# MatteoSoldini/metamorphic_testing_of_the_MUSICA_Algorithm_for_x_ray_image_processing

Hardware: AMD Instinct MI355X
Metric: megapixels/sec full MUSICA pipeline (higher is better)
Workload: dtype f32

## Files before the change

metamorphic_testing_of_the_musica_algorithm_for_x_ray_image_processing_amd/build.py:

```python
import os
import subprocess
import sys

HERE = os.path.dirname(os.path.abspath(__file__))
CSRC = os.path.join(HERE, "csrc")
LIB = os.path.join(HERE, "libmusica_hip.so")
CLI = os.path.join(HERE, "musica-standalone")
HIP_SOURCES = ["kernels_pyramid.hip", "kernels_expand_sd.hip", "kernels_analysis.hip", "kernels_gradation.hip", "kernels_clahe.hip", "kernels_bench.hip",
               "kernels_similarity.hip", "kernels_joint.hip", "kernels_displace.hip", "kernels_scales.hip", "kernels_ensemble.hip", "kernels_covariance.hip", "kernels_alteration.hip", "kernels_symmetry.hip", "kernels_export.hip", "musica_ctx.hip", "musica_study.hip"]
CPP_SOURCES = ["musica_io.cpp"]
HEADERS = ["musica_device.h", "kernels_common.h", "exact_math.h", "sdev_parts.h", "grad_parts.h", "launchers.h", "musica_ctx.h", os.path.join("..", "..", "include", "musica.h")]
NO_SLP = {"kernels_analysis.hip", "kernels_expand_sd.hip"}
FLAGS = ["--offload-arch=gfx950", "-O3", "-std=c++17", "-fPIC", "-ffp-contract=off", "-fno-fast-math", "-Wall", "-Wno-unused-function", "-Wno-unused-value", "-Wno-unused-result"]


def _hipcc():
    for cand in (os.environ.get("HIPCC"), "/opt/rocm/bin/hipcc", "hipcc"):
        if cand and (os.path.isabs(cand) and os.path.exists(cand) or not os.path.isabs(cand)):
            return cand
    return "hipcc"


def _stale(target, deps):
    if not os.path.exists(target):
        return True
    t = os.path.getmtime(target)
    return any(os.path.getmtime(d) > t for d in deps if os.path.exists(d))


def build(force=False, verbose=False):
    hipcc = _hipcc()
    objdir = os.path.join(HERE, "build")
    os.makedirs(objdir, exist_ok=True)
    headers = [os.path.normpath(os.path.join(CSRC, h)) for h in HEADERS]
# ... 105 lines not shown
```

metamorphic_testing_of_the_musica_algorithm_for_x_ray_image_processing_amd/csrc/exact_math.h:

```cpp
#pragma once

#include <math.h>
#include <stdint.h>

#if defined(__HIPCC__)
#define MUSICA_HD __host__ __device__ __forceinline__
#else
#define MUSICA_HD static inline
#endif

MUSICA_HD float musica_div25(float x) {
    const float y = 0.04f;
    const float q = x * y;
    const float r = fmaf(-25.0f, q, x);
    return r == r ? fmaf(r, y, q) : q;
}

MUSICA_HD int musica_noise_bin_exact(float cur) {
    if (cur != cur) return 0;
    if (cur == 0.0f) return 0;
    const float a = cur / 0.1f;
    if (a > 1.0f) return 0;
    return (int)(a * 2048.0f + 0.5f);
}
// ... 19 lines not shown
    return fmaf(r, h, s);
}
__device__ __forceinline__ bool musica_sqrt_core_ok(float x) {
    const uint32_t u = __float_as_uint(x);
    return u == 0u || (u - 0x0D800000u) < (0x7F800000u - 0x0D800000u);
}
__device__ __forceinline__ void musica_sqrt8(float s[8]) {
    uint32_t mx = 0u, mn = 0xFFFFFFFFu;
#pragma unroll
    for (int j = 0; j < 8; j++) {
        const uint32_t u = __float_as_uint(s[j]);
        mx = max(mx, u);
        mn = min(mn, u - 1u);
    }
    const bool ok = mx < 0x7F800000u && mn >= 0x0D800000u - 1u;
    if (__builtin_expect(ok, 1)) {
#pragma unroll
        for (int j = 0; j < 8; j++) s[j] = musica_sqrt_core(s[j]);
    } else {
#pragma unroll
        for (int j = 0; j < 8; j++) s[j] = sqrtf(s[j]);
    }
}
__device__ __forceinline__ float musica_sqrt(float x) {
    const float s = musica_sqrt_core(x);
    if (__builtin_expect(!musica_sqrt_core_ok(x), 0)) return sqrtf(x);
    return s;
}
#endif
```

metamorphic_testing_of_the_musica_algorithm_for_x_ray_image_processing_amd/csrc/kernels_analysis.hip:

```cpp
#include <stdlib.h>
#include <algorithm>
#include "kernels_common.h"
#include "exact_math.h"
#include "launchers.h"
#include "sdev_parts.h"

namespace musica {

__global__ void k_clear(uint32_t* __restrict__ minmax, uint32_t* __restrict__ noise_hist, uint32_t* __restrict__ grad_hist,
                        uint32_t* __restrict__ clahe_hist, int batch, uint32_t* __restrict__ grad_hist_b, uint32_t* __restrict__ gzero) {
    const int i = blockIdx.x * blockDim.x + threadIdx.x;
    const int nh = batch * 4 * MUSICA_NOISE_BINS, gh = batch * MUSICA_GRAD_BINS;
    const int ch = clahe_hist ? batch * MUSICA_CLAHE_TILES * MUSICA_CLAHE_TILES * MUSICA_CLAHE_BINS : 0;
    if (minmax && i < batch) { minmax[kMinMaxStride * i] = 0xFFFFFFFFu; minmax[kMinMaxStride * i + kMaxWord] = 0u; }
    if (noise_hist && i < nh) noise_hist[i] = 0u;
    if (grad_hist && i < gh) grad_hist[i] = 0u;
    if (grad_hist_b && i < gh) grad_hist_b[i] = 0u;
    if (gzero && i < batch) gzero[i] = 0u;
    if (i < ch) clahe_hist[i] = 0u;
}

__device__ __forceinline__ uint32_t wave_min(uint32_t v) {
#pragma unroll
    for (int o = 32; o >= 1; o >>= 1) v = min(v, (uint32_t)__shfl_xor((int)v, o));
// ... 104 lines not shown
    }
}

__device__ __forceinline__ bool same_float(float a, float b) { return __float_as_uint(a) == __float_as_uint(b) || (a != a && b != b); }
__global__ __launch_bounds__(256) void k_selftest_sqrt(unsigned long long* __restrict__ bad) {
    const uint64_t stride = (uint64_t)gridDim.x * blockDim.x;
    unsigned long long b0 = 0, b1 = 0, b2 = 0;
    for (uint64_t grp = (uint64_t)blockIdx.x * blockDim.x + threadIdx.x; grp < (1ull << 29); grp += stride) {
        float want[8], s[8], z[8];
#pragma unroll
        for (int j = 0; j < 8; j++) {
            const float x = __uint_as_float((uint32_t)(grp * 8 + j));
            want[j] = sqrtf(x);
            s[j] = x;
            z[j] = j == (int)(grp & 7) ? 0.0f : x;
            if (!same_float(musica_sqrt(x), want[j])) b0++;
        }
        musica_sqrt8(s);
        musica_sqrt8(z);
#pragma unroll
        for (int j = 0; j < 8; j++) {
            if (!same_float(s[j], want[j])) b1++;
            if (!same_float(z[j], j == (int)(grp & 7) ? 0.0f : want[j])) b2++;
        }
    }
    if (b0) atomicAdd(&bad[0], b0);
    if (b1) atomicAdd(&bad[1], b1);
    if (b2) atomicAdd(&bad[2], b2);
}
__global__ __launch_bounds__(256) void k_selftest_norm(unsigned long long* __restrict__ bad) {
    if (blockIdx.y < blockIdx.x) return;
    const float minv = (float)blockIdx.x, maxv = (float)blockIdx.y;
    const NormK nk = make_norm(minv, maxv);
    unsigned long long b = 0;
    for (uint32_t v = threadIdx.x; v < 65536u; v += blockDim.x)
        if (!same_float(norm_px(v, nk), norm_px(v, minv, maxv - minv))) b++;
    if (b) atomicAdd(&bad[3], b);
}

__global__ __launch_bounds__(256) void k_normalize(const uint16_t* __restrict__ px, float* __restrict__ out, int N, int pitch,
                                                   size_t plane, const uint32_t* __restrict__ minmax, int min_chain_exact) {
    const int img = blockIdx.z;
    float minv, maxv;
    chain_scalars(minmax, img, min_chain_exact, minv, maxv);
    const NormK nk = make_norm(minv, maxv);
    const uint16_t* p = px + (size_t)img * N * N;
// ... 150 lines not shown
        const unsigned long long other = __shfl_xor(k, o);
        k = other > k ? other : k;
    }
    const int lane = threadIdx.x & 63, wv = threadIdx.x >> 6, nw = (blockDim.x + 63) >> 6;
    if (lane == 0) scratch[wv] = k;
    __syncthreads();
    unsigned long long r = 0ull;
    for (int i = 0; i < nw; i++) r = scratch[i] > r ? scratch[i] : r;
    __syncthreads();
    return r;
}

__device__ __forceinline__ void noise_curves_block(int level, int img, const uint32_t* __restrict__ hist, size_t hist_stride,
                                                   musica_hist_max_point* __restrict__ maxpts, DevCurve* __restrict__ curves,
                                                   const musica_contrast_params* __restrict__ cparams, int levels,
                                                   DevCurveLut* __restrict__ luts, const uint32_t* __restrict__ minmax, int min_chain_exact,
                                                   int* __restrict__ thr090) {
    __shared__ unsigned long long scratch[16];
    if (thr090 && level == levels - 1 && threadIdx.x == 255) {
        float minv, maxv;
        chain_scalars(minmax, img, min_chain_exact, minv, maxv);
        thr090[img] = norm_threshold_090(minv, maxv - minv);
    }
    __shared__ float sx[kCurveCap];
    __shared__ int sbucket[kCurveCap];
    __shared__ int sok;
    musica_hist_max_point mp;
    mp.maxValue = 0; mp.maxBin = 0;
    if (level <= MUSICA_CNR_LEVEL) {
        const uint32_t* h = hist + (size_t)img * hist_stride + (size_t)level * MUSICA_NOISE_BINS;
        unsigned long long k = 0ull;
        for (int i = threadIdx.x; i < MUSICA_NOISE_BINS; i += blockDim.x) {
            const unsigned long long ki = argmax_key(h[i], (uint32_t)i);
            k = ki > k ? ki : k;
        }
        k = block_max_u64(k, scratch);
        if (k) { mp.maxValue = (uint32_t)(k >> 32); mp.maxBin = 0xFFFFFFFFu - (uint32_t)(k & 0xFFFFFFFFull); }
    }
    DevCurve* c = curves + (size_t)img * levels + level;
    __shared__ float cx[kCurveCap], cy[kCurveCap];
    __shared__ int s_mono;
    if (threadIdx.x == 0) maxpts[(size_t)img * levels + level] = mp;
    const float low = cparams[level].lowContrastFactor, high = cparams[level].highContrastFactor;
    const bool constant = (low == 1.0f);
    const int npts = constant ? 2 : 33;
    if ((int)threadIdx.x < kCurveCap) {
        const int i = threadIdx.x;
        float x = 0.0f, y = 0.0f;
        if (constant) {
            if (i == 0) { x = 0.0f; y = high; }
            if (i == 1) { x = 1.0f; y = high; }
        } else if (i < 33) {
            const float p = (float)mp.maxBin * (1.0f / (float)MUSICA_NOISE_BINS) * kMaxNoiseValue;
            const int seg = i / 11;
            const uint32_t k = (uint32_t)(i - seg * 11);
            if (seg == 0) bezier_point(0.0f, 1.0f, p * 4.0f / 5.0f, low, p, low, k, x, y);
            else if (seg == 1) bezier_point(p, low, p * 6.0f / 5.0f, low, p * 7.0f / 5.0f, low * 4.0f / 5.0f, k, x, y);
            else bezier_point(p * 7.0f / 5.0f, low * 4.0f / 5.0f, p * 2.0f, 1.0f, 1.0f, 1.0f, k, x, y);
        }
        cx[i] = x;
        cy[i] = y;
    }
    __syncthreads();
    curve_store_parallel(c, cx, cy, &s_mono, npts, 0.0f, 0.0f, 0.0f);
    if (level >= MUSICA_COARSER_LEVELS_START) return;
    __syncthreads();
    DevCurveLut* lut = luts + (size_t)img * MUSICA_COARSER_LEVELS_START + level;
    const int count = npts;
    const float range = cx[kLutTailFirst - 1] * 1.25f;
    const float inv_w = (float)kLutBuckets / range;
    __shared__ int scoarse[kCurveCap];
    if (threadIdx.x == 0) sok = (s_mono && count == kLutPoints && range > 0.0f && inv_w < 3.0e38f && cx[0] == 0.0f) ? 1 : 0;
    if ((int)threadIdx.x < kCurveCap) {
        const float x = cx[threadIdx.x];
        sx[threadIdx.x] = x;
        const float kf = x * inv_w;
        sbucket[threadIdx.x] = ((int)threadIdx.x < count && kf < (float)kLutBuckets) ? (int)kf : kLutBuckets;
        const float cf = fminf(x * 256.0f, (float)(kLutCoarse - 1));
        scoarse[threadIdx.x] = (int)cf;
    }
    __syncthreads();
    if ((int)threadIdx.x < count) {
        const bool inside = sbucket[threadIdx.x] < kLutBuckets;
        if (inside != ((int)threadIdx.x < kLutTailFirst)) sok = 0;
    }
    for (int k = threadIdx.x; k < kLutBuckets + kLutCoarse; k += blockDim.x) {
        const bool fine = k < kLutBuckets;
        const int kb = fine ? k : k - kLutBuckets;
        const int first = fine ? 0 : kLutTailFirst;
        int jlo = first, inb = 0;
        float xa = __builtin_huge_valf(), xb = __builtin_huge_valf();
        for (int i = first; i < count && i < kCurveCap; i++) {
            const int b = fine ? sbucket[i] : scoarse[i];
            if (b < kb) jlo++;
            else if (b == kb) {
                if (inb == 0) xa = sx[i];
                else if (inb == 1) xb = sx[i];
                inb++;
            }
        }
        if (inb > 2) sok = 0;
        lut->bucket[k] = make_float4(__int_as_float(jlo * 16), xa, xb, 0.0f);
    }
    if ((int)threadIdx.x <= kLutPoints) {
        const int j = threadIdx.x;
        float4 sg = make_float4(0.0f, 0.0f, 0.0f, 0.0f);
        if (j == 0) sg = make_float4(cx[0], cy[0], 0.0f, 0.0f);
        else if (j < count) sg = make_float4(cx[j - 1], cy[j - 1], (cy[j] - cy[j - 1]) / (cx[j] - cx[j - 1]), 0.0f);
        lut->seg[j] = sg;
    }
    __syncthreads();
    if (threadIdx.x == 0) {
        lut->inv_w = inv_w;
        lut->ok = (uint32_t)sok;
        lut->pad0 = lut->pad1 = 0;
    }
}

__global__ __launch_bounds__(256) void k_noise_curves(const uint32_t* __restrict__ hist, size_t hist_stride,
                                                      musica_hist_max_point* __restrict__ maxpts, DevCurve* __restrict__ curves,
                                                      const musica_contrast_params* __restrict__ cparams, int levels,
                                                      DevCurveLut* __restrict__ luts, const uint32_t* __restrict__ minmax, int min_chain_exact,
                                                      int* __restrict__ thr090, int lev0) {
    noise_curves_block(lev0 + (int)blockIdx.x, blockIdx.y, hist, hist_stride, maxpts, curves, cparams, levels, luts, minmax, min_chain_exact, thr090);
}

__global__ __launch_bounds__(256) void k_curves_cnr(const uint32_t* __restrict__ hist, size_t hist_stride,
                                                    musica_hist_max_point* __restrict__ maxpts, DevCurve* __restrict__ curves,
                                                    const musica_contrast_params* __restrict__ cparams, int levels,
                                                    DevCurveLut* __restrict__ luts, const float* __restrict__ sdev, float* __restrict__ cnr,
                                                    int S, int pitch, size_t plane, int tiles_x, const uint32_t* __restrict__ minmax,
                                                    int min_chain_exact, int* __restrict__ thr090, int lev0) {
    const int img = blockIdx.y;
    const int nlev = levels - lev0;
    if ((int)blockIdx.x < nlev) {
        noise_curves_block(lev0 + (int)blockIdx.x, img, hist, hist_stride, maxpts, curves, cparams, levels, luts, minmax, min_chain_exact, thr090);
        return;
    }
// ... 237 lines not shown
```

metamorphic_testing_of_the_musica_algorithm_for_x_ray_image_processing_amd/csrc/kernels_common.h:

```cpp
#pragma once

#include "musica_device.h"
#include "exact_math.h"

namespace musica {

__device__ __forceinline__ float from_left_lane(float v) {
    const int s = __builtin_bit_cast(int, v);
    return __builtin_bit_cast(float, __builtin_amdgcn_update_dpp(s, s, 0x138, 0xF, 0xF, true));
}
__device__ __forceinline__ float from_right_lane(float v) {
    const int s = __builtin_bit_cast(int, v);
    return __builtin_bit_cast(float, __builtin_amdgcn_update_dpp(s, s, 0x130, 0xF, 0xF, true));
}

typedef int v4i __attribute__((ext_vector_type(4)));
typedef float v4f __attribute__((ext_vector_type(4)));
typedef float v2f __attribute__((ext_vector_type(2)));
__device__ v4f llvm_buffer_load_v4f32(v4i rsrc, int voffset, int soffset, int aux) __asm("llvm.amdgcn.raw.buffer.load.v4f32");
__device__ v2f llvm_buffer_load_v2f32(v4i rsrc, int voffset, int soffset, int aux) __asm("llvm.amdgcn.raw.buffer.load.v2f32");
__device__ float llvm_buffer_load_f32(v4i rsrc, int voffset, int soffset, int aux) __asm("llvm.amdgcn.raw.buffer.load.f32");
__device__ void llvm_buffer_store_v4f32(v4f data, v4i rsrc, int voffset, int soffset, int aux) __asm("llvm.amdgcn.raw.buffer.store.v4f32");
__device__ short llvm_buffer_load_i16(v4i rsrc, int voffset, int soffset, int aux) __asm("llvm.amdgcn.raw.buffer.load.i16");
__device__ void llvm_buffer_store_i16(short data, v4i rsrc, int voffset, int soffset, int aux) __asm("llvm.amdgcn.raw.buffer.store.i16");
// ... 196 lines not shown
    return 0.0f;
}

__device__ __forceinline__ void curve_finish(DevCurve* c) {
    const int count = (int)c->count;
    uint32_t mono = 1;
    for (int i = 0; i < kCurveCap; i++) {
        if (i + 1 < count) {
            c->m[i] = (c->y[i + 1] - c->y[i]) / (c->x[i + 1] - c->x[i]);
            if (!(c->x[i] <= c->x[i + 1])) mono = 0;
        } else {
            c->m[i] = 0.0f;
        }
        if (i >= count) {
            c->x[i] = 0.0f;
            c->y[i] = 0.0f;
        }
    }
    if (count > 0 && !(c->x[0] == c->x[0])) mono = 0;
    if (count > 63) mono = 0;
    c->monotone = mono;
}

__device__ __forceinline__ float interpolate(float from, float to, float percent) {
    float difference = to - from;
    return from + (difference * percent);
}

__device__ __forceinline__ void generate_curve(DevCurve* c, uint32_t& n, float sx, float sy, float mx, float my,
                                               float ex, float ey, uint32_t steps) {
    for (uint32_t i = 0; i < steps; i++) {
        float t = (float)i / 10.0f;
        float xa = interpolate(sx, mx, t);
        float ya = interpolate(sy, my, t);
        float xb = interpolate(mx, ex, t);
        float yb = interpolate(my, ey, t);
        c->x[n] = interpolate(xa, xb, t);
        c->y[n] = interpolate(ya, yb, t);
        n++;
    }
}

__device__ __forceinline__ void bezier_point(float sx, float sy, float mx, float my, float ex, float ey, uint32_t k, float& x, float& y) {
    const float t = (float)k / 10.0f;
    const float xa = interpolate(sx, mx, t);
    const float ya = interpolate(sy, my, t);
    const float xb = interpolate(mx, ex, t);
    const float yb = interpolate(my, ey, t);
    x = interpolate(xa, xb, t);
    y = interpolate(ya, yb, t);
}

__device__ __forceinline__ void curve_store_parallel(DevCurve* c, const float* sx, const float* sy, int* s_mono, int count, float t0, float ta, float t1) {
    const int i = threadIdx.x;
    if (i == 0) *s_mono = 1;
    __syncthreads();
    if (i < kCurveCap) {
        float m = 0.0f;
        if (i + 1 < count) {
            m = (sy[i + 1] - sy[i]) / (sx[i + 1] - sx[i]);
            if (!(sx[i] <= sx[i + 1])) *s_mono = 0;
        }
        if (i == 0 && count > 0 && !(sx[0] == sx[0])) *s_mono = 0;
        c->x[i] = sx[i];
        c->y[i] = sy[i];
        c->m[i] = m;
    }
    __syncthreads();
    if (i == 0) {
        c->count = (uint32_t)count;
        c->monotone = (*s_mono && count <= 63) ? 1u : 0u;
        c->t0 = t0; c->ta = ta; c->t1 = t1;
        c->pad = 0;
    }
}
// ... 21 lines not shown
```

metamorphic_testing_of_the_musica_algorithm_for_x_ray_image_processing_amd/csrc/kernels_pyramid.hip:

```cpp
#include <stdlib.h>
#include "kernels_common.h"
#include "sdev_parts.h"
#include "launchers.h"

#ifndef MUSICA_PYRAMID_SD_ONLY
#define MUSICA_PYRAMID_FULL 1
#endif

namespace musica {

struct LaneCfg {
    int c;
    bool active;
    bool left_mirror;
    bool last_active;
    bool lane0, lane63;
    uint32_t off;
    uint32_t off_l;
    uint32_t off_r;
    uint32_t coff;
    uint32_t coff_l;
    uint32_t coff_r;
};

// ... 487 lines not shown
    r = c > highCnr ? highFactor : r;
    r = c < lowCnr ? lowFactor : r;
    return r;
}
__device__ __forceinline__ float nr_factor(float c, float lowCnr, float lowFactor, float highCnr, float highFactor) {
    if (c < lowCnr) return lowFactor;
    else if (c > highCnr) return highFactor;
    const float m = (highFactor - lowFactor) / (highCnr - lowCnr);
    return m * c + lowFactor;
}

template <int GAIN>
__device__ __forceinline__ float gain_of(float s, float high, const CurveLds& t) {
    if (GAIN == GAIN_CONST) return high;
    if (GAIN == GAIN_RANGE) {
        if (s == 0.0f) return high;
        if (s >= 0.0f && s <= 1.0f) return 0.0f * s + high;
        return 0.0f;
    }
    return curve_eval(t, s);
}

struct LutLds {
    float4 bucket[kLutBuckets + kLutCoarse];
    float4 seg[kLutPoints + 1];
    float inv_w;
    uint32_t ok;
};
template <bool LUTOK>
__device__ __forceinline__ float curve_eval_lut(const CurveLds& t, const LutLds& lut, float s) {
    if (!LUTOK) return curve_eval(t, s);
    const float sf = fminf(s, 2.0f);
    const float kf = sf * lut.inv_w;
    const bool in_fine = kf < (float)kLutBuckets;
    const float tsel = in_fine ? kf : fminf(sf * 256.0f, (float)(kLutCoarse - 1));
    const int idx = max((int)tsel + (in_fine ? 0 : kLutBuckets), 0);
    const float4 e = lut.bucket[idx];
    const int joff = __float_as_int(e.x) + (e.y < sf ? 16 : 0) + (e.z < sf ? 16 : 0);
    const float4 g = *reinterpret_cast<const float4*>(reinterpret_cast<const char*>(lut.seg) + joff);
    const float r = g.z * (sf - g.x) + g.y;
    return sf < 0.0f ? 0.0f : r;
}

constexpr int kChSlots = 4, kChCopies = 2;
#ifndef MUSICA_SD_W
#define MUSICA_SD_W 3
#endif
#ifndef MUSICA_SD_CH_W
#define MUSICA_SD_CH_W 2
#endif
struct BRow {
    float v[8];
    float e0, e1;
};
__device__ __forceinline__ void sdev_from_band(const BRow& r0, const BRow& r1, const BRow& r2, const BRow& r3, const BRow& r4, bool lane0, bool lane63, float (&s)[8]) {
    float q[8];
#pragma unroll
    for (int j = 0; j < 8; j++) q[j] = sum5(r0.v[j] * r0.v[j], r1.v[j] * r1.v[j], r2.v[j] * r2.v[j], r3.v[j] * r3.v[j], r4.v[j] * r4.v[j]);
    const float qe0 = sum5(r0.e0 * r0.e0, r1.e0 * r1.e0, r2.e0 * r2.e0, r3.e0 * r3.e0, r4.e0 * r4.e0);
    const float qe1 = sum5(r0.e1 * r0.e1, r1.e1 * r1.e1, r2.e1 * r2.e1, r3.e1 * r3.e1, r4.e1 * r4.e1);
    float a6 = from_left_lane(q[6]), a7 = from_left_lane(q[7]);
    float b0 = from_right_lane(q[0]), b1 = from_right_lane(q[1]);
    if (lane0) { a6 = qe0; a7 = qe1; }
    if (lane63) { b0 = qe0; b1 = qe1; }
    s[0] = sum5(a6, a7, q[0], q[1], q[2]);
    s[1] = sum5(a7, q[0], q[1], q[2], q[3]);
    s[2] = sum5(q[0], q[1], q[2], q[3], q[4]);
    s[3] = sum5(q[1], q[2], q[3], q[4], q[5]);
    s[4] = sum5(q[2], q[3], q[4], q[5], q[6]);
    s[5] = sum5(q[3], q[4], q[5], q[6], q[7]);
    s[6] = sum5(q[4], q[5], q[6], q[7], b0);
    s[7] = sum5(q[5], q[6], q[7], b0, b1);
#pragma unroll
    for (int j = 0; j < 8; j++) s[j] = musica_div25(s[j]);
    musica_sqrt8(s);
}
template <int GAIN, bool NR, bool GH, bool LUTOK, bool CNR48, bool CH = false, bool SD = false>
__device__ __forceinline__ bool expand_march(const ExpandArgs& a, const CurveLds& tab, const LutLds& lut, uint32_t* lh, int img, uint32_t* lc = nullptr,
                                             uint32_t tx0 = 0u, uint32_t ty0 = 0u) {
    constexpr int kGhCopies = 4, kGhStride = MUSICA_GRAD_BINS + 8;
    const float nr_m = (a.highFactor - a.lowFactor) / (a.highCnr - a.lowCnr);
    const int lane = threadIdx.x & 63;
    const Tile tile = xcd_tile(a.swz);
    const int seg = __builtin_amdgcn_readfirstlane((int)(tile.segblock * kWavesPerBlock + (threadIdx.x >> 6)));
    const int k0 = seg * a.rows_per_wave;
    bool saw_zero = false;
    if (k0 < a.Sc) {
    const int k1 = min(k0 + a.rows_per_wave, a.Sc);
    const int S = a.S;
    const int cnrScale = GH ? 8 : a.cnrScale;
    const Buf bb = make_buf(a.band + (size_t)img * a.plane, a.plane * 4);
    const Buf sb = make_buf((GAIN != GAIN_CONST ? a.sdev : a.band) + (size_t)img * a.plane, a.plane * 4);
    const Buf ob = make_buf(a.recon + (size_t)img * a.plane, a.plane * 4);
    const Buf pb = make_buf(a.prev + (size_t)img * a.cplane, a.cplane * 4);
    const Buf wb = !GH ? bb : make_buf(a.le090 + (size_t)img * a.Sc * (S / 8), (size_t)a.Sc * (S / 8) * 2);
    const float* cnr = NR ? a.cnr + (size_t)img * a.cnrPlane : nullptr;
    const LaneCfg g = make_cfg(tile.strip, lane, S);
    const uint32_t rb = (uint32_t)a.pitch * 4u, crb = (uint32_t)a.cpitch * 4u;
    const uint32_t moff = g.off == kOob ? kOob : (uint32_t)g.c >> 2, mrb = (uint32_t)S >> 2;
    const int cxs[2] = {g.active ? g.c / cnrScale : 0, g.active ? (g.c + 4) / cnrScale : 0};
    const uint32_t border = 100u, lim = (uint32_t)S - border;
    uint32_t colin = 0u;
    if (GH) {
#pragma unroll
        for (int j = 0; j < 8; j++)
            if (g.active && (uint32_t)(g.c + j) > border && (uint32_t)(g.c + j) < lim) colin |= 1u << j;
    }
    uint32_t* lhc = lh + (GH ? (lane & (kGhCopies - 1)) * kGhStride : 0);
    const float fS = (float)S;
    uint32_t chx = 0u;
    if (CH) {
#pragma unroll
        for (int j = 0; j < 8; j++) chx |= (min(f2u((float)(g.c + j) / fS * (float)MUSICA_CLAHE_TILES) - tx0, 1u)) << j;
    }
    uint32_t* lcc = CH ? lc + (lane & (kChCopies - 1)) * (kChSlots * MUSICA_CLAHE_BINS) : nullptr;

    auto row_phase = [&](const int ph, float* b, const float* src, const float* sd, const float* low, const float* f, const uint32_t le_t,
                         const int kk, const uint32_t w_cnr, const uint32_t w_dark_or_ramp, const bool one_ramp, const bool one_dark) __attribute__((always_inline)) {
#pragma unroll
        for (int j = 0; j < 8; j++) {
            float p = src[j] * (GAIN == GAIN_CURVE ? curve_eval_lut<LUTOK>(tab, lut, sd[j]) : gain_of<GAIN>(GAIN != GAIN_CONST ? sd[j] : 0.0f, a.high, tab));
            if (NR) p = p * f[j];
            b[j] = low[j] + p;
        }
        store8_nt(ob, g.off + (uint32_t)(2 * kk + ph) * rb, b);
        if (GH) {
            const uint32_t dark = le_t >> (8 * ph);
            const uint32_t y = (uint32_t)(2 * kk + ph);
            const uint32_t m = (y > border && y < lim) ? colin : 0u;
            const uint32_t chy = CH ? min(f2u((float)y / fS * (float)MUSICA_CLAHE_TILES) - ty0, 1u) : 0u;
#pragma unroll
            for (int j = 0; j < 8; j++) {
                const float cur = b[j];
                saw_zero = saw_zero || (cur == 0.0f);
                const uint32_t bin = min((uint32_t)(int)fminf(fmaxf(cur * (float)MUSICA_GRAD_BINS, -1.0f), 2048.0f), (uint32_t)MUSICA_GRAD_BINS);
                const bool le090 = ((dark >> j) & 1u) != 0u;
                const uint32_t w = ((m >> j) & 1u) * (le090 ? w_dark_or_ramp : w_cnr);
                atomicAdd(&lhc[bin], w);
                if (CH) {
                    const float scaled = cur * (float)(MUSICA_CLAHE_BINS - 1) + 0.5f;
                    const bool inrange = scaled > -1.0f && scaled < (float)MUSICA_CLAHE_BINS;
                    if (((m >> j) & 1u) && inrange && (one_ramp || (one_dark && le090)))
                        atomicAdd(&lcc[((((chx >> j) & 1u) * 2u + chy) * MUSICA_CLAHE_BINS) + (uint32_t)(int)scaled], 1u);
                }
            }
        }
    };
    if constexpr (SD) {
        const uint32_t off_e = g.lane0 ? g.off_l : g.off_r;
        auto load_brow = [&](BRow& r, const int y, const bool wanted) __attribute__((always_inline)) {
            const uint32_t row_off = (wanted && y >= 0 && y < S) ? (uint32_t)y * rb : kOob;
            load8(r.v, bb, (g.off + row_off) | ((g.off | row_off) & kOob));
            const float2 e = bload2(bb, (off_e + row_off) | ((off_e | row_off) & kOob));
            r.e0 = e.x; r.e1 = e.y;
        };
        CRow c0, c1, cn;
        load_crow(c0, pb, (uint32_t)coarse_of_fine(2 * k0 - 2, S) * crb, g);
        load_crow(c1, pb, (uint32_t)k0 * crb, g);
// ... 122 lines not shown
                }
            }
        }
        const CnrClass kc = classify_cnr(cnr_pair);
        const uint32_t w_cnr = kc.ramp ? kc.w_ramp : 0u, w_dark_or_ramp = kc.ramp ? kc.w_ramp : (kc.high ? 100u : 0u);
        const float r6 = cnr_pair / 6.0f;
        const bool one_ramp = CH && kc.ramp && (((r6 * r6) * (r6 * r6)) * r6 == 1.0f);
        const bool one_dark = CH && !kc.ramp && kc.high;
        row_phase(0, be, be, se, lowE, fe, le, k, w_cnr, w_dark_or_ramp, one_ramp, one_dark);
        load8(be, bb, goff_n + (uint32_t)(2 * kn) * rb);
        if (GAIN != GAIN_CONST) load8(se, sb, goff_n + (uint32_t)(2 * kn) * rb);
        row_phase(1, bo, bo, so, lowO, fo, le, k, w_cnr, w_dark_or_ramp, one_ramp, one_dark);
        le = le_n;
    }
    }
    return saw_zero;
}

template <int GAIN, bool NR, bool GH, int W = 1, bool CH = false, bool SD = false>
__global__ __launch_bounds__(kBlockThreads, W) void k_expand_fast(ExpandArgs a) {
    __shared__ CurveLds tab;
    __shared__ __attribute__((aligned(16))) LutLds lut;
    constexpr int kGhCopies = 4, kGhStride = MUSICA_GRAD_BINS + 8;
    __shared__ uint32_t lh[GH ? kGhCopies * kGhStride : 1];
    __shared__ uint32_t lc[CH ? kChCopies * kChSlots * MUSICA_CLAHE_BINS : 1];
    const int img = blockIdx.z;
    if (GH)
        for (int i = threadIdx.x; i < kGhCopies * kGhStride; i += blockDim.x) lh[i] = 0u;
    uint32_t tx0 = 0u, ty0 = 0u;
    if (CH) {
        for (int i = threadIdx.x; i < kChCopies * kChSlots * MUSICA_CLAHE_BINS; i += blockDim.x) lc[i] = 0u;
        const Tile t = xcd_tile(a.swz);
        tx0 = f2u((float)(t.strip * kStripCols) / (float)a.S * (float)MUSICA_CLAHE_TILES);
        ty0 = f2u((float)(t.segblock * kWavesPerBlock * a.rows_per_wave * 2) / (float)a.S * (float)MUSICA_CLAHE_TILES);
    }
    if (GAIN == GAIN_CURVE) {
        const DevCurve* cv = a.curves + (size_t)img * a.curve_stride;
        const DevCurveLut* lv = a.luts + (size_t)img * MUSICA_COARSER_LEVELS_START;
        curve_to_lds(tab, cv);
        for (int i = threadIdx.x; i < kLutBuckets + kLutCoarse; i += blockDim.x) lut.bucket[i] = lv->bucket[i];
        for (int i = threadIdx.x; i <= kLutPoints; i += blockDim.x) lut.seg[i] = lv->seg[i];
        if (threadIdx.x == 0) { lut.inv_w = lv->inv_w; lut.ok = lv->ok; }
        __syncthreads();
    }
    const bool lut_ok = GAIN != GAIN_CURVE || __builtin_amdgcn_readfirstlane((int)lut.ok) != 0;
    const bool cnr48 = !NR || GH || a.cnrScale == 4 || a.cnrScale == 8;
    bool saw_zero;
    if (lut_ok && cnr48) saw_zero = expand_march<GAIN, NR, GH, true, true, CH, SD>(a, tab, lut, lh, img, lc, tx0, ty0);
    else if (lut_ok) saw_zero = expand_march<GAIN, NR, GH, true, NR && !GH ? false : true, CH, SD>(a, tab, lut, lh, img, lc, tx0, ty0);
    else if (cnr48) saw_zero = expand_march<GAIN, NR, GH, GAIN != GAIN_CURVE, true, CH, SD>(a, tab, lut, lh, img, lc, tx0, ty0);
    else saw_zero = expand_march<GAIN, NR, GH, GAIN != GAIN_CURVE, NR && !GH ? false : true, CH, SD>(a, tab, lut, lh, img, lc, tx0, ty0);
    if (GH) {
        if (saw_zero) atomicOr(&a.gzero[img], 1u);
        __syncthreads();
        uint32_t* gh = a.ghist + (size_t)img * MUSICA_GRAD_BINS;
        for (int i = threadIdx.x; i < MUSICA_GRAD_BINS; i += blockDim.x) {
            uint32_t v = 0u;
#pragma unroll
            for (int k = 0; k < kGhCopies; k++) v += lh[k * kGhStride + i];
            if (v) atomicAdd(&gh[i], v);
        }
        if (CH) {
            uint32_t* ch = a.chist + (size_t)img * MUSICA_CLAHE_TILES * MUSICA_CLAHE_TILES * MUSICA_CLAHE_BINS;
            for (int i = threadIdx.x; i < kChSlots * MUSICA_CLAHE_BINS; i += blockDim.x) {
                const uint32_t slot = (uint32_t)i / MUSICA_CLAHE_BINS, tx = tx0 + (slot >> 1), ty = ty0 + (slot & 1u);
                uint32_t v = 0u;
#pragma unroll
                for (int k = 0; k < kChCopies; k++) v += lc[k * kChSlots * MUSICA_CLAHE_BINS + i];
                if (v && tx < (uint32_t)MUSICA_CLAHE_TILES && ty < (uint32_t)MUSICA_CLAHE_TILES)
                    atomicAdd(&ch[(tx * MUSICA_CLAHE_TILES + ty) * MUSICA_CLAHE_BINS + ((uint32_t)i % MUSICA_CLAHE_BINS)], v);
            }
        }
    }
}

__device__ __forceinline__ void curve_to_lds_2d(CurveLds& tab, const DevCurve* __restrict__ src) {
    const int tid = threadIdx.y * blockDim.x + threadIdx.x;
    for (int i = tid; i < kCurveCap; i += blockDim.x * blockDim.y) {
        tab.x[i] = src->x[i]; tab.y[i] = src->y[i]; tab.m[i] = src->m[i];
    }
    if (tid == 0) { tab.count = src->count; tab.monotone = src->monotone; }
}
// ... 260 lines not shown
```

metamorphic_testing_of_the_musica_algorithm_for_x_ray_image_processing_amd/csrc/musica_device.h:

```cpp
#pragma once

#include <hip/hip_runtime.h>
#include <stdint.h>

#include "../../include/musica.h"

namespace musica {

__device__ constexpr float W0 = 0.1f, W1 = 0.25f, W2 = 0.3f, W3 = 0.25f, W4 = 0.1f;

constexpr int kLaneCols = 8;
constexpr int kStripCols = 64 * kLaneCols;
constexpr int kWavesPerBlock = 4;
constexpr int kBlockThreads = 64 * kWavesPerBlock;

constexpr float kMaxNoiseValue = 0.1f;
constexpr float kMaxCnrValue = 256.0f;
constexpr int kHistArea = 16;
constexpr int kMinMaxStride = 32;
constexpr int kMaxWord = 16;
constexpr int kCurveCap = 64;

struct DevCurve {
    float x[kCurveCap];
    float y[kCurveCap];
    float m[kCurveCap];
    uint32_t count;
    uint32_t monotone;
    float t0, ta, t1;
    uint32_t pad;
};

constexpr int kLutBuckets = 256;
constexpr int kLutCoarse = 258;
constexpr int kLutTailFirst = 23;
constexpr int kLutPoints = 33;
struct DevCurveLut {
    float inv_w;
    uint32_t ok;
    uint32_t pad0, pad1;
    float4 bucket[kLutBuckets + kLutCoarse];
    float4 seg[kLutPoints + 1];
};

struct LevelDesc {
    int S;
    int pitch;
    size_t plane;
};

constexpr int kSdevRunLevelsMax = 4;
struct SdevRunLevel {
    const float* band;
    float* sdev;
    uint32_t* hist;
    size_t plane;
    int S, pitch, strips, first;
    int rows;
    int blocks;
};
struct SdevRunLevels {
    SdevRunLevel l[kSdevRunLevelsMax];
    int n;
    int swz;
// ... 23 lines not shown
```

metamorphic_testing_of_the_musica_algorithm_for_x_ray_image_processing_amd/csrc/sdev_parts.h:

```cpp
#pragma once

#include "kernels_common.h"
#include "exact_math.h"

namespace musica {

constexpr int kHistCopies = 3;
constexpr int kHistCopyStride = MUSICA_NOISE_BINS + 8;
constexpr int kHistLdsWords = kHistCopies * kHistCopyStride + 64;
__device__ __forceinline__ void hist_lds_clear(uint32_t* lh) {
    for (int i = threadIdx.x; i < kHistLdsWords; i += blockDim.x) lh[i] = 0u;
}
__device__ __forceinline__ void hist_lds_flush(const uint32_t* lh, uint32_t* __restrict__ gh) {
    for (int i = threadIdx.x; i < MUSICA_NOISE_BINS; i += blockDim.x) {
        uint32_t v = 0u;
#pragma unroll
        for (int k = 0; k < kHistCopies; k++) v += lh[k * kHistCopyStride + i];
        if (v) atomicAdd(&gh[i], v);
    }
}

struct SRow {
    float q[8];
    float l0, l1;
// ... 65 lines not shown
    acc = acc + d;
    acc = acc + e;
    return acc;
}

__device__ __forceinline__ void sdev_values(const SRow& r0, const SRow& r1, const SRow& r2, const SRow& r3, const SRow& r4, const SCfg& g, float (&s)[8]) {
    float q[8];
#pragma unroll
    for (int j = 0; j < 8; j++) q[j] = sum5(r0.q[j], r1.q[j], r2.q[j], r3.q[j], r4.q[j]);
    const float ql0 = sum5(r0.l0, r1.l0, r2.l0, r3.l0, r4.l0), ql1 = sum5(r0.l1, r1.l1, r2.l1, r3.l1, r4.l1);
    const float qh0 = sum5(r0.h0, r1.h0, r2.h0, r3.h0, r4.h0), qh1 = sum5(r0.h1, r1.h1, r2.h1, r3.h1, r4.h1);
    float a6 = from_left_lane(q[6]), a7 = from_left_lane(q[7]);
    float b0 = from_right_lane(q[0]), b1 = from_right_lane(q[1]);
    if (g.lane0) { a6 = ql0; a7 = ql1; }
    if (g.lane63) { b0 = qh0; b1 = qh1; }
    s[0] = sum5(a6, a7, q[0], q[1], q[2]);
    s[1] = sum5(a7, q[0], q[1], q[2], q[3]);
    s[2] = sum5(q[0], q[1], q[2], q[3], q[4]);
    s[3] = sum5(q[1], q[2], q[3], q[4], q[5]);
    s[4] = sum5(q[2], q[3], q[4], q[5], q[6]);
    s[5] = sum5(q[3], q[4], q[5], q[6], q[7]);
    s[6] = sum5(q[4], q[5], q[6], q[7], b0);
    s[7] = sum5(q[5], q[6], q[7], b0, b1);
#pragma unroll
    for (int j = 0; j < 8; j++) s[j] = musica_div25(s[j]);
    musica_sqrt8(s);
}
template <bool A8>
__device__ __forceinline__ void sdev_store(const float (&s)[8], const SCfg& g, float* __restrict__ drow, const Buf& db, uint32_t row_off) {
    if (A8) {
        bstore4(db, (g.off0 + row_off) | (g.off0 & kOob), make_float4(s[0], s[1], s[2], s[3]));
        bstore4(db, (g.off1 + row_off) | (g.off1 & kOob), make_float4(s[4], s[5], s[6], s[7]));
    } else if (g.valid == 8) {
        *reinterpret_cast<float4*>(drow + g.c) = make_float4(s[0], s[1], s[2], s[3]);
        *reinterpret_cast<float4*>(drow + g.c + 4) = make_float4(s[4], s[5], s[6], s[7]);
    } else {
#pragma unroll
        for (int j = 0; j < 8; j++)
            if (j < g.valid) drow[g.c + j] = s[j];
    }
}

template <bool HIST, bool A8>
__device__ __forceinline__ void sdev_row(const SRow& r0, const SRow& r1, const SRow& r2, const SRow& r3, const SRow& r4, const SCfg& g, int S,
                                         int y, int cov, float* __restrict__ drow, const Buf& db, uint32_t row_off, uint32_t* lh,
                                         unsigned long long (&alive)[8], const unsigned long long (&start)[8], bool store = true) {
    float s[8];
    sdev_values(r0, r1, r2, r3, r4, g, s);
    if (store) sdev_store<A8>(s, g, drow, db, row_off);
// ... 140 lines not shown
```

Measured before the change: 115,200.

## Key curve LUT on float exponent bits and fuse div25+sqrt range check

Replaces the two-level bucket LUT for the gain curve (fine buckets scaled by inv_w plus a coarse tail) with a single table indexed by the float's bit pattern shifted right, starting at a per-curve base key. This removes a float multiply, a compare and a select from each curve evaluation, and the kernel copies only the used entries into LDS. The LDS table grows to 1160 entries, which may lower occupancy. It also adds musica_rms25_8, which checks the range once for all 8 values before doing the exact divide-by-25 and fast sqrt, and drops the clamp on the histogram bin by shifting the histogram base by one word so a bin of -1 stays in bounds.

```diff
diff --git a/metamorphic_testing_of_the_musica_algorithm_for_x_ray_image_processing_amd/build.py b/metamorphic_testing_of_the_musica_algorithm_for_x_ray_image_processing_amd/build.py
--- a/metamorphic_testing_of_the_musica_algorithm_for_x_ray_image_processing_amd/build.py
+++ b/metamorphic_testing_of_the_musica_algorithm_for_x_ray_image_processing_amd/build.py
@@ -9,7 +9,7 @@
 HIP_SOURCES = ["kernels_pyramid.hip", "kernels_expand_sd.hip", "kernels_analysis.hip", "kernels_gradation.hip", "kernels_clahe.hip", "kernels_bench.hip",
                "kernels_similarity.hip", "kernels_joint.hip", "kernels_displace.hip", "kernels_scales.hip", "kernels_ensemble.hip", "kernels_covariance.hip", "kernels_alteration.hip", "kernels_symmetry.hip", "kernels_export.hip", "musica_ctx.hip", "musica_study.hip"]
 CPP_SOURCES = ["musica_io.cpp"]
-HEADERS = ["musica_device.h", "kernels_common.h", "exact_math.h", "sdev_parts.h", "grad_parts.h", "launchers.h", "musica_ctx.h", os.path.join("..", "..", "include", "musica.h")]
+HEADERS = ["musica_device.h", "kernels_common.h", "exact_math.h", "curve_lut.h", "sdev_parts.h", "grad_parts.h", "launchers.h", "musica_ctx.h", os.path.join("..", "..", "include", "musica.h")]
 NO_SLP = {"kernels_analysis.hip", "kernels_expand_sd.hip"}
 FLAGS = ["--offload-arch=gfx950", "-O3", "-std=c++17", "-fPIC", "-ffp-contract=off", "-fno-fast-math", "-Wall", "-Wno-unused-function", "-Wno-unused-value", "-Wno-unused-result"]
 
diff --git a/metamorphic_testing_of_the_musica_algorithm_for_x_ray_image_processing_amd/csrc/curve_lut.h b/metamorphic_testing_of_the_musica_algorithm_for_x_ray_image_processing_amd/csrc/curve_lut.h
--- /dev/null
+++ b/metamorphic_testing_of_the_musica_algorithm_for_x_ray_image_processing_amd/csrc/curve_lut.h
@@ -0,0 +1,99 @@
+#pragma once
+
+#include <math.h>
+#include <stdint.h>
+#include <string.h>
+
+#include "exact_math.h"
+
+namespace musica {
+
+constexpr int kLutPoints = 33;
+constexpr int kLutShift = 17;
+constexpr int kLutKeyTop = 0x40000000 >> kLutShift;
+constexpr int kLutCap = 1160;
+
+MUSICA_HD int32_t musica_float_bits(float f) {
+#if defined(__HIP_DEVICE_COMPILE__)
+    return __float_as_int(f);
+#else
+    int32_t i;
+    memcpy(&i, &f, sizeof i);
+    return i;
+#endif
+}
+MUSICA_HD float musica_bits_float(int32_t i) {
+#if defined(__HIP_DEVICE_COMPILE__)
+    return __int_as_float(i);
+#else
+    float f;
+    memcpy(&f, &i, sizeof f);
+    return f;
+#endif
+}
+MUSICA_HD float musica_lut_clamp(float s) { return s < 2.0f ? s : 2.0f; }
+MUSICA_HD int musica_lut_key_clamped(float sf) { return musica_float_bits(sf) >> kLutShift; }
+MUSICA_HD int musica_lut_key(float s) { return musica_lut_key_clamped(musica_lut_clamp(s)); }
+MUSICA_HD int musica_lut_index(int key, int base) { return (key > base ? key : base) - base; }
+
+MUSICA_HD float interpolate(float from, float to, float percent) {
+    float difference = to - from;
+    return from + (difference * percent);
+}
+MUSICA_HD void bezier_point(float sx, float sy, float mx, float my, float ex, float ey, uint32_t k, float& x, float& y) {
+    const float t = (float)k / 10.0f;
+    const float xa = interpolate(sx, mx, t);
+    const float ya = interpolate(sy, my, t);
+    const float xb = interpolate(mx, ex, t);
+    const float yb = interpolate(my, ey, t);
+    x = interpolate(xa, xb, t);
+    y = interpolate(ya, yb, t);
+}
+MUSICA_HD void musica_contrast_point(uint32_t maxBin, float low, int i, float& x, float& y) {
+    const float p = (float)maxBin * (1.0f / 2048.0f) * 0.1f;
+    const int seg = i / 11;
+    const uint32_t k = (uint32_t)(i - seg * 11);
+    if (seg == 0) bezier_point(0.0f, 1.0f, p * 4.0f / 5.0f, low, p, low, k, x, y);
+    else if (seg == 1) bezier_point(p, low, p * 6.0f / 5.0f, low, p * 7.0f / 5.0f, low * 4.0f / 5.0f, k, x, y);
+    else bezier_point(p * 7.0f / 5.0f, low * 4.0f / 5.0f, p * 2.0f, 1.0f, 1.0f, 1.0f, k, x, y);
+}
+
+MUSICA_HD int musica_lut_base(const float* x) { return musica_lut_key(x[1]) - 1; }
+MUSICA_HD int musica_lut_entries(int base) {
+    const int n = kLutKeyTop - base + 1;
+    return (base >= 0 && n <= kLutCap) ? n : 0;
+}
+MUSICA_HD int musica_lut_slot(float x, int base) { return musica_lut_index(musica_lut_key(x), base); }
+constexpr int kLutSlotSentinel = 0x7FFFFFFF;
+template <class F4>
+MUSICA_HD int musica_lut_entry(const float* x, const int* b, int count, int k, F4& e) {
+    int jlo = 0;
+    for (int step = 32; step >= 1; step >>= 1) {
+        const int probe = jlo + step;
+        if (probe <= count && b[probe - 1] < k) jlo = probe;
+    }
+    const bool ia = b[jlo] == k, ib = b[jlo + 1] == k, ic = b[jlo + 2] == k;
+    e.x = musica_bits_float(jlo * 16);
+    e.y = ia ? x[jlo] : (float)INFINITY;
+    e.z = ib ? x[jlo + 1] : (float)INFINITY;
+    e.w = 0.0f;
+    return (ia ? 1 : 0) + (ib ? 1 : 0) + (ic ? 1 : 0);
+}
+template <class F4>
+MUSICA_HD void musica_lut_segment(const float* x, const float* y, int count, int j, F4& sg) {
+    sg.x = sg.y = sg.z = sg.w = 0.0f;
+    if (j == 0) { sg.x = x[0]; sg.y = y[0]; }
+    else if (j < count) { sg.x = x[j - 1]; sg.y = y[j - 1]; sg.z = (y[j] - y[j - 1]) / (x[j] - x[j - 1]); }
+}
+template <class F4>
+MUSICA_HD float musica_lut_eval(const F4* bucket, const F4* seg, int base, float s) {
+    const float sf = musica_lut_clamp(s);
+    const int idx = musica_lut_index(musica_lut_key_clamped(sf), base);
+    const F4 e = *reinterpret_cast<const F4*>(reinterpret_cast<const char*>(bucket) + (uint32_t)idx * 16u);
+    const int joff = musica_float_bits(e.x) + (e.y < sf ? 16 : 0) + (e.z < sf ? 16 : 0);
+    const F4 g = *reinterpret_cast<const F4*>(reinterpret_cast<const char*>(seg) + joff);
+    const float r = g.z * (sf - g.x) + g.y;
+    return sf < 0.0f ? 0.0f : r;
+}
+
+}
diff --git a/metamorphic_testing_of_the_musica_algorithm_for_x_ray_image_processing_amd/csrc/exact_math.h b/metamorphic_testing_of_the_musica_algorithm_for_x_ray_image_processing_amd/csrc/exact_math.h
--- a/metamorphic_testing_of_the_musica_algorithm_for_x_ray_image_processing_amd/csrc/exact_math.h
+++ b/metamorphic_testing_of_the_musica_algorithm_for_x_ray_image_processing_amd/csrc/exact_math.h
@@ -65,6 +65,27 @@
         for (int j = 0; j < 8; j++) s[j] = sqrtf(s[j]);
     }
 }
+__device__ __forceinline__ void musica_rms25_8(float s[8]) {
+    uint32_t mx = 0u, mn = 0xFFFFFFFFu;
+#pragma unroll
+    for (int j = 0; j < 8; j++) {
+        const uint32_t u = __float_as_uint(s[j]);
+        mx = max(mx, u);
+        mn = min(mn, u - 1u);
+    }
+    const bool ok = mx < 0x7F800000u && mn >= 0x10000000u - 1u;
+    if (__builtin_expect(ok, 1)) {
+#pragma unroll
+        for (int j = 0; j < 8; j++) {
+            const float q = s[j] * 0.04f;
+            const float r = fmaf(-25.0f, q, s[j]);
+            s[j] = musica_sqrt_core(fmaf(r, 0.04f, q));
+        }
+    } else {
+#pragma unroll
+        for (int j = 0; j < 8; j++) s[j] = sqrtf(s[j] / 25.0f);
+    }
+}
 __device__ __forceinline__ float musica_sqrt(float x) {
     const float s = musica_sqrt_core(x);
     if (__builtin_expect(!musica_sqrt_core_ok(x), 0)) return sqrtf(x);
diff --git a/metamorphic_testing_of_the_musica_algorithm_for_x_ray_image_processing_amd/csrc/kernels_analysis.hip b/metamorphic_testing_of_the_musica_algorithm_for_x_ray_image_processing_amd/csrc/kernels_analysis.hip
--- a/metamorphic_testing_of_the_musica_algorithm_for_x_ray_image_processing_amd/csrc/kernels_analysis.hip
+++ b/metamorphic_testing_of_the_musica_algorithm_for_x_ray_image_processing_amd/csrc/kernels_analysis.hip
@@ -150,6 +150,26 @@
         for (int j = 0; j < 8; j++) {
             if (!same_float(s[j], want[j])) b1++;
             if (!same_float(z[j], j == (int)(grp & 7) ? 0.0f : want[j])) b2++;
+        }
+        const float repl[3] = {0.0f, __uint_as_float(0x03800000u) , __uint_as_float(0x7F800000u)};
+        float want25[8], r[8];
+#pragma unroll
+        for (int j = 0; j < 8; j++) {
+            r[j] = __uint_as_float((uint32_t)(grp * 8 + j));
+            want25[j] = sqrtf(r[j] / 25.0f);
+        }
+        musica_rms25_8(r);
+#pragma unroll
+        for (int j = 0; j < 8; j++)
+            if (!same_float(r[j], want25[j])) b1++;
+#pragma unroll
+        for (int k = 0; k < 3; k++) {
+#pragma unroll
+            for (int j = 0; j < 8; j++) r[j] = j == (int)(grp & 7) ? repl[k] : __uint_as_float((uint32_t)(grp * 8 + j));
+            musica_rms25_8(r);
+#pragma unroll
+            for (int j = 0; j < 8; j++)
+                if (!same_float(r[j], j == (int)(grp & 7) ? sqrtf(repl[k] / 25.0f) : want25[j])) b2++;
         }
     }
     if (b0) atomicAdd(&bad[0], b0);
@@ -346,8 +366,6 @@
         chain_scalars(minmax, img, min_chain_exact, minv, maxv);
         thr090[img] = norm_threshold_090(minv, maxv - minv);
     }
-    __shared__ float sx[kCurveCap];
-    __shared__ int sbucket[kCurveCap];
     __shared__ int sok;
     musica_hist_max_point mp;
     mp.maxValue = 0; mp.maxBin = 0;
@@ -375,12 +393,8 @@
             if (i == 0) { x = 0.0f; y = high; }
             if (i == 1) { x = 1.0f; y = high; }
         } else if (i < 33) {
-            const float p = (float)mp.maxBin * (1.0f / (float)MUSICA_NOISE_BINS) * kMaxNoiseValue;
-            const int seg = i / 11;
-            const uint32_t k = (uint32_t)(i - seg * 11);
-            if (seg == 0) bezier_point(0.0f, 1.0f, p * 4.0f / 5.0f, low, p, low, k, x, y);
-            else if (seg == 1) bezier_point(p, low, p * 6.0f / 5.0f, low, p * 7.0f / 5.0f, low * 4.0f / 5.0f, k, x, y);
-            else bezier_point(p * 7.0f / 5.0f, low * 4.0f / 5.0f, p * 2.0f, 1.0f, 1.0f, 1.0f, k, x, y);
+            static_assert(MUSICA_NOISE_BINS == 2048 && kMaxNoiseValue == 0.1f, "musica_contrast_point spells the noise mode out");
+            musica_contrast_point(mp.maxBin, low, i, x, y);
         }
         cx[i] = x;
         cy[i] = y;
@@ -391,53 +405,28 @@
     __syncthreads();
     DevCurveLut* lut = luts + (size_t)img * MUSICA_COARSER_LEVELS_START + level;
     const int count = npts;
-    const float range = cx[kLutTailFirst - 1] * 1.25f;
-    const float inv_w = (float)kLutBuckets / range;
-    __shared__ int scoarse[kCurveCap];
-    if (threadIdx.x == 0) sok = (s_mono && count == kLutPoints && range > 0.0f && inv_w < 3.0e38f && cx[0] == 0.0f) ? 1 : 0;
-    if ((int)threadIdx.x < kCurveCap) {
-        const float x = cx[threadIdx.x];
-        sx[threadIdx.x] = x;
-        const float kf = x * inv_w;
-        sbucket[threadIdx.x] = ((int)threadIdx.x < count && kf < (float)kLutBuckets) ? (int)kf : kLutBuckets;
-        const float cf = fminf(x * 256.0f, (float)(kLutCoarse - 1));
-        scoarse[threadIdx.x] = (int)cf;
-    }
-    __syncthreads();
-    if ((int)threadIdx.x < count) {
-        const bool inside = sbucket[threadIdx.x] < kLutBuckets;
-        if (inside != ((int)threadIdx.x < kLutTailFirst)) sok = 0;
-    }
-    for (int k = threadIdx.x; k < kLutBuckets + kLutCoarse; k += blockDim.x) {
-        const bool fine = k < kLutBuckets;
-        const int kb = fine ? k : k - kLutBuckets;
-        const int first = fine ? 0 : kLutTailFirst;
-        int jlo = first, inb = 0;
-        float xa = __builtin_huge_valf(), xb = __builtin_huge_valf();
-        for (int i = first; i < count && i < kCurveCap; i++) {
-            const int b = fine ? sbucket[i] : scoarse[i];
-            if (b < kb) jlo++;
-            else if (b == kb) {
-                if (inb == 0) xa = sx[i];
-                else if (inb == 1) xb = sx[i];
-                inb++;
-            }
-        }
-        if (inb > 2) sok = 0;
-        lut->bucket[k] = make_float4(__int_as_float(jlo * 16), xa, xb, 0.0f);
+    const int base = musica_lut_base(cx);
+    const int n = (s_mono && count == kLutPoints && cx[0] == 0.0f) ? musica_lut_entries(base) : 0;
+    __shared__ int sslot[kCurveCap];
+    if (threadIdx.x == 0) sok = n > 0 ? 1 : 0;
+    if ((int)threadIdx.x < kCurveCap) sslot[threadIdx.x] = (int)threadIdx.x < count ? musica_lut_slot(cx[threadIdx.x], base) : kLutSlotSentinel;
+    __syncthreads();
+    for (int k = threadIdx.x; k < n; k += blockDim.x) {
+        float4 e;
+        if (musica_lut_entry(cx, sslot, count, k, e) > 2) sok = 0;
+        lut->bucket[k] = e;
     }
     if ((int)threadIdx.x <= kLutPoints) {
-        const int j = threadIdx.x;
-        float4 sg = make_float4(0.0f, 0.0f, 0.0f, 0.0f);
-        if (j == 0) sg = make_float4(cx[0], cy[0], 0.0f, 0.0f);
-        else if (j < count) sg = make_float4(cx[j - 1], cy[j - 1], (cy[j] - cy[j - 1]) / (cx[j] - cx[j - 1]), 0.0f);
-        lut->seg[j] = sg;
+        float4 sg;
+        musica_lut_segment(cx, cy, count, (int)threadIdx.x, sg);
+        lut->seg[threadIdx.x] = sg;
     }
     __syncthreads();
     if (threadIdx.x == 0) {
-        lut->inv_w = inv_w;
+        lut->base = base;
         lut->ok = (uint32_t)sok;
-        lut->pad0 = lut->pad1 = 0;
+        lut->n = (uint32_t)n;
+        lut->pad0 = 0;
     }
 }
 
diff --git a/metamorphic_testing_of_the_musica_algorithm_for_x_ray_image_processing_amd/csrc/kernels_common.h b/metamorphic_testing_of_the_musica_algorithm_for_x_ray_image_processing_amd/csrc/kernels_common.h
--- a/metamorphic_testing_of_the_musica_algorithm_for_x_ray_image_processing_amd/csrc/kernels_common.h
+++ b/metamorphic_testing_of_the_musica_algorithm_for_x_ray_image_processing_amd/csrc/kernels_common.h
@@ -242,10 +242,6 @@
     c->monotone = mono;
 }
 
-__device__ __forceinline__ float interpolate(float from, float to, float percent) {
-    float difference = to - from;
-    return from + (difference * percent);
-}
 
 __device__ __forceinline__ void generate_curve(DevCurve* c, uint32_t& n, float sx, float sy, float mx, float my,
                                                float ex, float ey, uint32_t steps) {
@@ -261,16 +257,6 @@
     }
 }
 
-__device__ __forceinline__ void bezier_point(float sx, float sy, float mx, float my, float ex, float ey, uint32_t k, float& x, float& y) {
-    const float t = (float)k / 10.0f;
-    const float xa = interpolate(sx, mx, t);
-    const float ya = interpolate(sy, my, t);
-    const float xb = interpolate(mx, ex, t);
-    const float yb = interpolate(my, ey, t);
-    x = interpolate(xa, xb, t);
-    y = interpolate(ya, yb, t);
-}
-
 __device__ __forceinline__ void curve_store_parallel(DevCurve* c, const float* sx, const float* sy, int* s_mono, int count, float t0, float ta, float t1) {
     const int i = threadIdx.x;
     if (i == 0) *s_mono = 1;
diff --git a/metamorphic_testing_of_the_musica_algorithm_for_x_ray_image_processing_amd/csrc/kernels_pyramid.hip b/metamorphic_testing_of_the_musica_algorithm_for_x_ray_image_processing_amd/csrc/kernels_pyramid.hip
--- a/metamorphic_testing_of_the_musica_algorithm_for_x_ray_image_processing_amd/csrc/kernels_pyramid.hip
+++ b/metamorphic_testing_of_the_musica_algorithm_for_x_ray_image_processing_amd/csrc/kernels_pyramid.hip
@@ -533,24 +533,15 @@
 }
 
 struct LutLds {
-    float4 bucket[kLutBuckets + kLutCoarse];
+    float4 bucket[kLutCap];
     float4 seg[kLutPoints + 1];
-    float inv_w;
+    int32_t base;
     uint32_t ok;
 };
 template <bool LUTOK>
-__device__ __forceinline__ float curve_eval_lut(const CurveLds& t, const LutLds& lut, float s) {
+__device__ __forceinline__ float curve_eval_lut(const CurveLds& t, const LutLds& lut, int base, float s) {
     if (!LUTOK) return curve_eval(t, s);
-    const float sf = fminf(s, 2.0f);
-    const float kf = sf * lut.inv_w;
-    const bool in_fine = kf < (float)kLutBuckets;
-    const float tsel = in_fine ? kf : fminf(sf * 256.0f, (float)(kLutCoarse - 1));
-    const int idx = max((int)tsel + (in_fine ? 0 : kLutBuckets), 0);
-    const float4 e = lut.bucket[idx];
-    const int joff = __float_as_int(e.x) + (e.y < sf ? 16 : 0) + (e.z < sf ? 16 : 0);
-    const float4 g = *reinterpret_cast<const float4*>(reinterpret_cast<const char*>(lut.seg) + joff);
-    const float r = g.z * (sf - g.x) + g.y;
-    return sf < 0.0f ? 0.0f : r;
+    return musica_lut_eval(lut.bucket, lut.seg, base, s);
 }
 
 constexpr int kChSlots = 4, kChCopies = 2;
@@ -582,9 +573,7 @@
     s[5] = sum5(q[3], q[4], q[5], q[6], q[7]);
     s[6] = sum5(q[4], q[5], q[6], q[7], b0);
     s[7] = sum5(q[5], q[6], q[7], b0, b1);
-#pragma unroll
-    for (int j = 0; j < 8; j++) s[j] = musica_div25(s[j]);
-    musica_sqrt8(s);
+    musica_rms25_8(s);
 }
 template <int GAIN, bool NR, bool GH, bool LUTOK, bool CNR48, bool CH = false, bool SD = false>
 __device__ __forceinline__ bool expand_march(const ExpandArgs& a, const CurveLds& tab, const LutLds& lut, uint32_t* lh, int img, uint32_t* lc = nullptr,
@@ -596,6 +585,7 @@
     const int seg = __builtin_amdgcn_readfirstlane((int)(tile.segblock * kWavesPerBlock + (threadIdx.x >> 6)));
     const int k0 = seg * a.rows_per_wave;
     bool saw_zero = false;
+    const int lut_base = (GAIN == GAIN_CURVE && LUTOK) ? __builtin_amdgcn_readfirstlane(lut.base) : 0;
     if (k0 < a.Sc) {
     const int k1 = min(k0 + a.rows_per_wave, a.Sc);
     const int S = a.S;
@@ -617,7 +607,7 @@
         for (int j = 0; j < 8; j++)
             if (g.active && (uint32_t)(g.c + j) > border && (uint32_t)(g.c + j) < lim) colin |= 1u << j;
     }
-    uint32_t* lhc = lh + (GH ? (lane & (kGhCopies - 1)) * kGhStride : 0);
+    uint32_t* lhc = lh + (GH ? 1 + (lane & (kGhCopies - 1)) * kGhStride : 0);
     const float fS = (float)S;
     uint32_t chx = 0u;
     if (CH) {
@@ -630,7 +620,7 @@
                          const int kk, const uint32_t w_cnr, const uint32_t w_dark_or_ramp, const bool one_ramp, const bool one_dark) __attribute__((always_inline)) {
 #pragma unroll
         for (int j = 0; j < 8; j++) {
-            float p = src[j] * (GAIN == GAIN_CURVE ? curve_eval_lut<LUTOK>(tab, lut, sd[j]) : gain_of<GAIN>(GAIN != GAIN_CONST ? sd[j] : 0.0f, a.high, tab));
+            float p = src[j] * (GAIN == GAIN_CURVE ? curve_eval_lut<LUTOK>(tab, lut, lut_base, sd[j]) : gain_of<GAIN>(GAIN != GAIN_CONST ? sd[j] : 0.0f, a.high, tab));
             if (NR) p = p * f[j];
             b[j] = low[j] + p;
         }
@@ -644,7 +634,7 @@
             for (int j = 0; j < 8; j++) {
                 const float cur = b[j];
                 saw_zero = saw_zero || (cur == 0.0f);
-                const uint32_t bin = min((uint32_t)(int)fminf(fmaxf(cur * (float)MUSICA_GRAD_BINS, -1.0f), 2048.0f), (uint32_t)MUSICA_GRAD_BINS);
+                const int bin = (int)fminf(fmaxf(cur * (float)MUSICA_GRAD_BINS, -1.0f), (float)MUSICA_GRAD_BINS);
                 const bool le090 = ((dark >> j) & 1u) != 0u;
                 const uint32_t w = ((m >> j) & 1u) * (le090 ? w_dark_or_ramp : w_cnr);
                 atomicAdd(&lhc[bin], w);
@@ -813,11 +803,11 @@
     __shared__ CurveLds tab;
     __shared__ __attribute__((aligned(16))) LutLds lut;
     constexpr int kGhCopies = 4, kGhStride = MUSICA_GRAD_BINS + 8;
-    __shared__ uint32_t lh[GH ? kGhCopies * kGhStride : 1];
+    __shared__ uint32_t lh[GH ? kGhCopies * kGhStride + 1 : 1];
     __shared__ uint32_t lc[CH ? kChCopies * kChSlots * MUSICA_CLAHE_BINS : 1];
     const int img = blockIdx.z;
     if (GH)
-        for (int i = threadIdx.x; i < kGhCopies * kGhStride; i += blockDim.x) lh[i] = 0u;
+        for (int i = threadIdx.x; i < kGhCopies * kGhStride + 1; i += blockDim.x) lh[i] = 0u;
     uint32_t tx0 = 0u, ty0 = 0u;
     if (CH) {
         for (int i = threadIdx.x; i < kChCopies * kChSlots * MUSICA_CLAHE_BINS; i += blockDim.x) lc[i] = 0u;
@@ -829,9 +819,10 @@
         const DevCurve* cv = a.curves + (size_t)img * a.curve_stride;
         const DevCurveLut* lv = a.luts + (size_t)img * MUSICA_COARSER_LEVELS_START;
         curve_to_lds(tab, cv);
-        for (int i = threadIdx.x; i < kLutBuckets + kLutCoarse; i += blockDim.x) lut.bucket[i] = lv->bucket[i];
+        const int nlut = lv->ok ? min((int)lv->n, kLutCap) : 0;
+        for (int i = threadIdx.x; i < nlut; i += blockDim.x) lut.bucket[i] = lv->bucket[i];
         for (int i = threadIdx.x; i <= kLutPoints; i += blockDim.x) lut.seg[i] = lv->seg[i];
-        if (threadIdx.x == 0) { lut.inv_w = lv->inv_w; lut.ok = lv->ok; }
+        if (threadIdx.x == 0) { lut.base = lv->base; lut.ok = lv->ok; }
         __syncthreads();
     }
     const bool lut_ok = GAIN != GAIN_CURVE || __builtin_amdgcn_readfirstlane((int)lut.ok) != 0;
@@ -848,7 +839,7 @@
         for (int i = threadIdx.x; i < MUSICA_GRAD_BINS; i += blockDim.x) {
             uint32_t v = 0u;
 #pragma unroll
-            for (int k = 0; k < kGhCopies; k++) v += lh[k * kGhStride + i];
+            for (int k = 0; k < kGhCopies; k++) v += lh[1 + k * kGhStride + i];
             if (v) atomicAdd(&gh[i], v);
         }
         if (CH) {
diff --git a/metamorphic_testing_of_the_musica_algorithm_for_x_ray_image_processing_amd/csrc/musica_device.h b/metamorphic_testing_of_the_musica_algorithm_for_x_ray_image_processing_amd/csrc/musica_device.h
--- a/metamorphic_testing_of_the_musica_algorithm_for_x_ray_image_processing_amd/csrc/musica_device.h
+++ b/metamorphic_testing_of_the_musica_algorithm_for_x_ray_image_processing_amd/csrc/musica_device.h
@@ -4,6 +4,7 @@
 #include <stdint.h>
 
 #include "../../include/musica.h"
+#include "curve_lut.h"
 
 namespace musica {
 
@@ -31,15 +32,12 @@
     uint32_t pad;
 };
 
-constexpr int kLutBuckets = 256;
-constexpr int kLutCoarse = 258;
-constexpr int kLutTailFirst = 23;
-constexpr int kLutPoints = 33;
 struct DevCurveLut {
-    float inv_w;
+    int32_t base;
     uint32_t ok;
-    uint32_t pad0, pad1;
-    float4 bucket[kLutBuckets + kLutCoarse];
+    uint32_t n;
+    uint32_t pad0;
+    float4 bucket[kLutCap];
     float4 seg[kLutPoints + 1];
 };
 
diff --git a/metamorphic_testing_of_the_musica_algorithm_for_x_ray_image_processing_amd/csrc/sdev_parts.h b/metamorphic_testing_of_the_musica_algorithm_for_x_ray_image_processing_amd/csrc/sdev_parts.h
--- a/metamorphic_testing_of_the_musica_algorithm_for_x_ray_image_processing_amd/csrc/sdev_parts.h
+++ b/metamorphic_testing_of_the_musica_algorithm_for_x_ray_image_processing_amd/csrc/sdev_parts.h
@@ -111,9 +111,7 @@
     s[5] = sum5(q[3], q[4], q[5], q[6], q[7]);
     s[6] = sum5(q[4], q[5], q[6], q[7], b0);
     s[7] = sum5(q[5], q[6], q[7], b0, b1);
-#pragma unroll
-    for (int j = 0; j < 8; j++) s[j] = musica_div25(s[j]);
-    musica_sqrt8(s);
+    musica_rms25_8(s);
 }
 template <bool A8>
 __device__ __forceinline__ void sdev_store(const float (&s)[8], const SCfg& g, float* __restrict__ drow, const Buf& db, uint32_t row_off) {
```

After: 117,800, median of 6. +2.3%, better.
